# shiyao-li/NextBestPath

Measured on AMD Instinct MI355X. Metric: exploration steps/s (+ NBP maps/s) at 256x256, higher is better.
Workload: dtype f32

## Files before the change

### include/nbp_hip.h

```cpp
#ifndef NBP_HIP_H
#define NBP_HIP_H

#include <stddef.h>
#include <stdint.h>

#ifdef __cplusplus
extern "C" {
#endif

#define NBP_E_ARG      (-1)
#define NBP_E_WS       (-2)
#define NBP_E_SHAPE    (-3)

int nbp_abi_version(void);
int nbp_device_info(char* arch_host, int arch_len, int* cu_count_host);
int nbp_tuning_active(void);
int nbp_tuning_report(char* buf_host, int len);
int nbp_tile_kernel_symbol(int tile, char* buf_host, int len);

#define NBP_N_CONV 48

typedef struct nbp_weights nbp_weights;

size_t nbp_packed_weights_bytes(void);

int nbp_pack_weights(const void* const* w_host_array, const void* const* scale_host_array,
                     const void* const* shift_host_array, void* packed, size_t packed_bytes,
                     void* stream, nbp_weights** handle_out);
void nbp_free_weights(nbp_weights* handle);

size_t nbp_forward_workspace_bytes(int B, int S);

int nbp_forward_f32(const nbp_weights* handle, const float* x, int B, int S, float* out1,
                    float* out2, void* ws, size_t ws_bytes, void* stream);

typedef struct nbp_layer_timing {
    char name[48];
    double flops;
    float ms;
    int tile, split_k;
    long long M;
    int N, K;
} nbp_layer_timing;
int nbp_forward_timed_f32(const nbp_weights* handle, const float* x, int B, int S, float* out1,
                          float* out2, void* ws, size_t ws_bytes, void* stream,
                          nbp_layer_timing* timings_host, int max_entries, int* n_entries_host);

double nbp_forward_flops(int B, int S);

int nbp_pack_weights_bf16(const void* const* w_host_array, const void* const* scale_host_array,
                          const void* const* shift_host_array, void* packed, size_t packed_bytes,
                          void* stream, nbp_weights** handle_out);
// ... 29 lines not shown
int nbp_conv3x3_split_f32(const float* src0, int C0, const float* src1, int C1, int ups, int B, int H, int W,
                          const void* w_planes, const void* wamax, int N, const float* scale, const float* shift, int relu,
                          float* out, const void* amax_in_or_null, void* amax_out_or_null, int split_k, void* ws,
                          size_t ws_bytes, void* stream);
size_t nbp_conv_first_wgrad_workspace_bytes(void);
int nbp_conv_first_wgrad_f32(const float* x_nchw, int B, int H, int W, const float* dy, float* dw, void* ws, size_t ws_bytes, void* stream);
int nbp_prepack_weights_split(const void* descs_dev, int n, void* wamax_words, void* stream);
int nbp_prepack_desc_bytes(void);
int nbp_pack_conv_weight_split_prezeroed(const float* w_oihw, int N, int C, int ksize, int c_total, void* dst_planes,
                                         void* wamax_zeroed, void* stream);
int nbp_pack_conv_weight_split_dgrad_known(const float* w_oihw, int N, int C, int c_total, void* dst_planes, const void* wamax_known,
                                           void* stream);
int nbp_pack_upconv_weight_split_dgrad(const float* w_oihw, int N, int C, void* dst_planes, void* wamax_out, void* stream);
size_t nbp_upconv_split_dgrad_workspace_bytes(int B, int H, int W, int N, int C);
int nbp_upconv3x3_split_dgrad_f32(const float* dy, int N, int B, int H, int W, const void* planes, const void* wamax, int C,
                                  const float* scale, const float* shift, float* dx, const void* amax_in, void* amax_out_or_null,
                                  void* ws, size_t ws_bytes, void* stream);
size_t nbp_upconv_wgrad_split_workspace_bytes(int B, int Hs, int Ws, int C, int N);
int nbp_upconv_wgrad_split_f32(const float* x, int C, int B, int Hs, int Ws, const float* dy, int N, float* dw,
                               const void* amax_x, const void* amax_y, void* ws, size_t ws_bytes, void* stream);
int nbp_conv1x1_split_f32(const float* src, int C, long long M, const void* w_planes, const void* wamax, int N,
                          const float* scale, const float* shift, int relu, float* out, const void* amax_in, void* stream);
int nbp_pack_conv1x1_weight_split_dgrad(const float* w_nc, int N, int C, void* dst_planes, void* wamax_out, void* stream);
int nbp_pack_conv_weight_split_dgrad(const float* w_oihw, int N, int C, int c_total, void* dst_planes, void* wamax_out, void* stream);

int nbp_conv_bn_part_rows(int B, int H, int W);
int nbp_conv3x3_split_bn_f32(const float* src0, int C0, const float* src1, int C1, int ups, int B, int H, int W,
                             const void* w_planes, const void* wamax, int N, const float* scale, const float* shift, int relu,
                             float* out, const void* amax_in_or_null, void* amax_out_or_null, int split_k, void* ws,
                             size_t ws_bytes, double* bn_part, int* bn_rows, void* stream);
int nbp_upconv3x3_split_bn_f32(const float* src, int C, int B, int H, int W, const void* planes_up, const void* wamax_up, int N,
                               const float* scale, const float* shift, int relu, float* out, const void* amax_in_or_null,
                               void* amax_out_or_null, int split_k, void* ws, size_t ws_bytes, double* bn_part, int* bn_rows,
                               void* stream);
int nbp_pack_conv_weight_split_h1(const float* w_oihw, int N, int C, int ksize, const float* scale_or_null, int c_off,
                                  int c_total, void* dst_planes, void* wamax_out, void* stream);
int nbp_pack_conv_weight_split_prezeroed_h1(const float* w_oihw, int N, int C, int ksize, int c_total, void* dst_planes,
                                            void* wamax_zeroed, void* stream);
int nbp_pack_conv_weight_split_dgrad_h1(const float* w_oihw, int N, int C, int c_total, void* dst_planes, void* wamax_out, void* stream);
int nbp_pack_conv_weight_split_dgrad_known_h1(const float* w_oihw, int N, int C, int c_total, void* dst_planes, const void* wamax_known,
                                              void* stream);
int nbp_pack_upconv_weight_split_h1(const float* w_oihw, int N, int C, void* dst_planes, void* wamax_out, void* stream);
int nbp_pack_upconv_weight_split_dgrad_h1(const float* w_oihw, int N, int C, void* dst_planes, void* wamax_out, void* stream);
int nbp_pack_conv1x1_weight_split_dgrad_h1(const float* w_nc, int N, int C, void* dst_planes, void* wamax_out, void* stream);
int nbp_prepack_weights_split_h1(const void* descs_dev, int n, void* wamax_words, void* stream);
int nbp_conv3x3_split_f32_h1(const float* src0, int C0, const float* src1, int C1, int ups, int B, int H, int W,
// ... 390 lines not shown
```

### nextbestpath_amd/_lib.py

```python
from __future__ import annotations

import ctypes as C
import os
import threading

HERE = os.path.dirname(os.path.abspath(__file__))
LIB_PATH = os.path.join(HERE, "libnbp_hip.so")

_vp, _i, _ll, _f, _sz, _d = C.c_void_p, C.c_int, C.c_longlong, C.c_float, C.c_size_t, C.c_double

SIGNATURES = {
    "nbp_abi_version": (_i, []),
    "nbp_device_info": (_i, [C.c_char_p, _i, C.POINTER(_i)]),
    "nbp_tuning_active": (_i, []),
    "nbp_tuning_report": (_i, [C.c_char_p, _i]),
    "nbp_tile_kernel_symbol": (_i, [_i, C.c_char_p, _i]),
    "nbp_packed_weights_bytes": (_sz, []),
    "nbp_pack_weights": (_i, [C.POINTER(_vp), C.POINTER(_vp), C.POINTER(_vp), _vp, _sz, _vp, C.POINTER(_vp)]),
    "nbp_free_weights": (None, [_vp]),
    "nbp_forward_workspace_bytes": (_sz, [_i, _i]),
    "nbp_forward_f32": (_i, [_vp, _vp, _i, _i, _vp, _vp, _vp, _sz, _vp]),
    "nbp_forward_flops": (_d, [_i, _i]),
    "nbp_conv_igemm_f32": (_i, [_vp, _i, _vp, _i, _i, _i, _i, _i, _i, _vp, _i, _vp, _vp, _i, _vp, _i, _i, _vp,
                                _sz, _vp]),
# ... 97 lines not shown
SIGNATURES["nbp_amax_f32"] = (_i, [_vp, _ll, _vp, _vp])
SIGNATURES["nbp_pack_upconv_weight_split"] = (_i, [_vp, _i, _i, _vp, _vp, _vp])
SIGNATURES["nbp_upconv3x3_split_f32"] = (_i, [_vp, _i, _i, _i, _i, _vp, _vp, _i, _vp, _vp, _i, _vp, _vp, _vp, _i, _vp, _sz, _vp])
SIGNATURES["nbp_conv_split_workspace_bytes"] = SIGNATURES["nbp_conv_igemm_workspace_bytes"]
SIGNATURES["nbp_conv_split_planned_workspace_bytes"] = (_sz, [_i, _i, _i, _i, _i, _i, _vp])
SIGNATURES["nbp_conv_split_planned_workspace_bytes_k"] = (_sz, [_i, _i, _i, _i, _i, _i, _i, _vp])
SIGNATURES["nbp_conv3x3_split_f32"] = (_i, [_vp, _i, _vp, _i, _i, _i, _i, _i, _vp, _vp, _i, _vp, _vp, _i, _vp, _vp, _vp, _i, _vp,
                                            _sz, _vp])
SIGNATURES["nbp_pack_upconv_weight_split_dgrad"] = (_i, [_vp, _i, _i, _vp, _vp, _vp])
SIGNATURES["nbp_upconv_split_dgrad_workspace_bytes"] = (_sz, [_i, _i, _i, _i, _i])
SIGNATURES["nbp_upconv3x3_split_dgrad_f32"] = (_i, [_vp, _i, _i, _i, _i, _vp, _vp, _i, _vp, _vp, _vp, _vp, _vp, _vp, _sz, _vp])
SIGNATURES["nbp_upconv_wgrad_split_workspace_bytes"] = (_sz, [_i, _i, _i, _i, _i])
SIGNATURES["nbp_upconv_wgrad_split_f32"] = (_i, [_vp, _i, _i, _i, _i, _vp, _i, _vp, _vp, _vp, _vp, _sz, _vp])
SIGNATURES["nbp_pack_conv_weight_split_prezeroed"] = (_i, [_vp, _i, _i, _i, _i, _vp, _vp, _vp])
SIGNATURES["nbp_pack_conv_weight_split_dgrad_known"] = (_i, [_vp, _i, _i, _i, _vp, _vp, _vp])
SIGNATURES["nbp_prepack_weights_split"] = (_i, [_vp, _i, _vp, _vp])
SIGNATURES["nbp_prepack_desc_bytes"] = (_i, [])
SIGNATURES["nbp_rowscale_amax_f32"] = (_i, [_vp, _vp, _ll, _i, _vp, _vp, _vp])
SIGNATURES["nbp_conv_first_linear_f32"] = (_i, [_vp, _i, _i, _i, _vp, _vp, _vp, _vp, _vp])
SIGNATURES["nbp_conv_first_wgrad_workspace_bytes"] = (_sz, [])
SIGNATURES["nbp_conv_first_wgrad_f32"] = (_i, [_vp, _i, _i, _i, _vp, _vp, _vp, _sz, _vp])
SIGNATURES["nbp_conv1x1_split_f32"] = (_i, [_vp, _i, _ll, _vp, _vp, _i, _vp, _vp, _i, _vp, _vp, _vp])
SIGNATURES["nbp_pack_conv1x1_weight_split_dgrad"] = (_i, [_vp, _i, _i, _vp, _vp, _vp])
SIGNATURES["nbp_pack_conv_weight_split_dgrad"] = (_i, [_vp, _i, _i, _i, _vp, _vp, _vp])
SIGNATURES["nbp_conv_bn_part_rows"] = (_i, [_i, _i, _i])
SIGNATURES["nbp_conv3x3_split_bn_f32"] = (_i, [_vp, _i, _vp, _i, _i, _i, _i, _i, _vp, _vp, _i, _vp, _vp, _i, _vp, _vp, _vp, _i, _vp,
                                               _sz, _vp, C.POINTER(_i), _vp])
SIGNATURES["nbp_upconv3x3_split_bn_f32"] = (_i, [_vp, _i, _i, _i, _i, _vp, _vp, _i, _vp, _vp, _i, _vp, _vp, _vp, _i, _vp, _sz, _vp,
                                                 C.POINTER(_i), _vp])
SIGNATURES["nbp_bn_train_forward_part4_f32"] = (_i, [_vp, _ll, _i, _vp, _vp, _f, _f, _vp, _vp, _i, _vp, _vp, _vp, _vp, _vp, _i, _vp, _i, _vp, _vp])
for _n in ("nbp_pack_conv_weight_split", "nbp_pack_conv_weight_split_prezeroed", "nbp_pack_conv_weight_split_dgrad",
           "nbp_pack_conv_weight_split_dgrad_known", "nbp_pack_upconv_weight_split", "nbp_pack_upconv_weight_split_dgrad",
           "nbp_pack_conv1x1_weight_split_dgrad", "nbp_prepack_weights_split", "nbp_conv3x3_split_f32", "nbp_conv3x3_split_bn_f32",
           "nbp_upconv3x3_split_f32", "nbp_upconv3x3_split_bn_f32", "nbp_upconv3x3_split_dgrad_f32", "nbp_conv1x1_split_f32",
           "nbp_upconv_wgrad_split_f32", "nbp_conv_wgrad_split_f32"):
    SIGNATURES[_n + "_h1"] = SIGNATURES[_n]
SIGNATURES["nbp_conv_igemm_bf16"] = SIGNATURES["nbp_conv_igemm_f32"]
SIGNATURES["nbp_conv_igemm_bf16_workspace_bytes"] = SIGNATURES["nbp_conv_igemm_workspace_bytes"]
SIGNATURES["nbp_pack_conv_weight_bf16"] = SIGNATURES["nbp_pack_conv_weight"]
SIGNATURES["nbp_f32_to_bf16"] = (_i, [_vp, _ll, _vp, _vp])
SIGNATURES["nbp_bf16_to_f32"] = (_i, [_vp, _ll, _vp, _vp])
_fpp, _ipp = C.POINTER(_f), C.POINTER(_i)
SIGNATURES["nbp_scene_fill_workspace_bytes"] = (_sz, [_fpp, _ipp, _i, _ll, _d])
SIGNATURES["nbp_scene_fill_cells_f32"] = (_i, [_vp, _ll, _vp, _fpp, _ipp, _i, _d, _i, C.c_uint, _vp, _vp, _vp, _sz, _vp])
SIGNATURES["nbp_scene_gather_f32"] = (_i, [_vp, _vp, _i, _i, _vp, _ll, _vp, _vp])
SIGNATURES["nbp_scene_coverage_workspace_bytes"] = (_sz, [_fpp, _ipp, _i, _d])
# ... 160 lines not shown
```

### nextbestpath_amd/csrc/nbp_forward.hip

```cpp
#include "common.h"
#include "nbp_internal.h"
#include <stdio.h>
#include <stdlib.h>
#include <string.h>

namespace {

enum Kind { K_FIRST, K_CONV3, K_ATT_G, K_ATT_X, K_PSI, K_FINAL };
struct LayerSpec { Kind kind; int cin, cout, k; };

struct Table {
    LayerSpec L[NBP_N_CONV];
    size_t w_off[NBP_N_CONV];
    size_t s_off[NBP_N_CONV], t_off[NBP_N_CONV];
    size_t total_floats;
    size_t w3_off[NBP_N_CONV];
    size_t w3u_off[NBP_N_CONV];
    bool is_up[NBP_N_CONV];
    int up_rank[NBP_N_CONV];
    size_t total3_bytes;
    size_t wup16_off[NBP_N_CONV], total_up16_bytes;
    size_t w1_off[NBP_N_CONV];
    int gate_rank[NBP_N_CONV];
    Table() {
// ... 74 lines not shown
    for (long long i = (long long)blockIdx.x * blockDim.x + threadIdx.x; i < n; i += (long long)gridDim.x * blockDim.x)
        dst[i] = v;
}
int fill_f32(float* dst, float v, long long n, hipStream_t st) {
    fill_f32_kernel<<<nbp_ew_grid(n, 256), 256, 0, st>>>(dst, v, n);
    return nbp_launch_status();
}

}

struct nbp_weights {
    const void* w[NBP_N_CONV];
    const float* scale[NBP_N_CONV];
    const float* shift[NBP_N_CONV];
    int bf16;
    const void* w3[NBP_N_CONV];
    const unsigned* wamax[NBP_N_CONV];
    const void* wup16[NBP_N_CONV];
    const void* w1[NBP_N_CONV];
    const unsigned* wamax1[NBP_N_CONV];
    const void* w3u[NBP_N_CONV];
    const unsigned* wamax_u[NBP_N_CONV];
    int split;
};

extern "C" int nbp_abi_version(void) {
    NBP_ENTER(); return NBP_ABI_VERSION; }

extern "C" int nbp_device_info(char* arch_host, int arch_len, int* cu_count_host) {
    NBP_ENTER();
    int dev = 0;
    hipError_t e = hipGetDevice(&dev);
    if (e != hipSuccess) return (int)e;
    hipDeviceProp_t p;
    e = hipGetDeviceProperties(&p, dev);
    if (e != hipSuccess) return (int)e;
    if (arch_host && arch_len > 0) { strncpy(arch_host, p.gcnArchName, arch_len - 1); arch_host[arch_len - 1] = 0; }
    if (cu_count_host) *cu_count_host = p.multiProcessorCount;
    return 0;
}

extern "C" size_t nbp_packed_weights_bytes(void) { return table().total_floats * sizeof(float); }

static int pack_weights_impl(const void* const* w_host_array, const void* const* scale_host_array,
                             const void* const* shift_host_array, void* packed, size_t packed_bytes, void* stream,
                             nbp_weights** handle_out, bool bf16, bool split = false) {
    NBP_RETURN_IF(!w_host_array || !scale_host_array || !shift_host_array || !packed || !handle_out, NBP_E_ARG);
    const Table& T = table();
    NBP_RETURN_IF(packed_bytes < T.total_floats * sizeof(float) + (split ? T.total3_bytes : 0) + (bf16 ? T.total_up16_bytes : 0),
                  NBP_E_WS);
    for (int i = 0; i < NBP_N_CONV; ++i) {
        NBP_RETURN_IF(!w_host_array[i] || !scale_host_array[i], NBP_E_ARG);
        NBP_RETURN_IF(T.L[i].kind != K_ATT_X && !shift_host_array[i], NBP_E_ARG);
    }
    hipStream_t st = (hipStream_t)stream;
    float* base = (float*)packed;
    nbp_weights* h = (nbp_weights*)calloc(1, sizeof(nbp_weights));
    NBP_RETURN_IF(!h, NBP_E_ARG);
    h->bf16 = bf16 ? 1 : 0;
    h->split = split ? 1 : 0;
    char* base3 = (char*)packed + T.total_floats * sizeof(float);
    int rc = 0;
    for (int i = 0; i < NBP_N_CONV && !rc; ++i) {
        const LayerSpec& s = T.L[i];
        const float* w = (const float*)w_host_array[i];
        const float* sc = (const float*)scale_host_array[i];
        const float* sh = (const float*)shift_host_array[i];
        float* wd = base + T.w_off[i];
        float* sd = base + T.s_off[i];
        float* td = base + T.t_off[i];
        h->w[i] = wd; h->scale[i] = sd; h->shift[i] = td;
        switch (s.kind) {
            case K_FIRST: case K_FINAL:
                rc = copy_f32(w, wd, (long long)s.cout * s.cin * s.k * s.k, st);
                if (!rc) rc = copy_f32(sc, sd, s.cout, st);
                if (!rc) rc = copy_f32(sh, td, s.cout, st);
                break;
            case K_PSI:
                rc = copy_f32(w, wd, s.cin, st);
                if (!rc) rc = copy_f32(sc, sd, 1, st);
                if (!rc) rc = copy_f32(sh, sd + 1, 1, st);
                if (!rc) rc = copy_f32(sh, td, 1, st);
                break;
// ... 57 lines not shown
                             false);
}

extern "C" int nbp_pack_weights_bf16(const void* const* w_host_array, const void* const* scale_host_array,
                                     const void* const* shift_host_array, void* packed, size_t packed_bytes,
                                     void* stream, nbp_weights** handle_out) {
    NBP_ENTER();
    return pack_weights_impl(w_host_array, scale_host_array, shift_host_array, packed, packed_bytes, stream, handle_out,
                             true);
}

extern "C" size_t nbp_packed_weights_bytes_split(void) { return table().total_floats * sizeof(float) + table().total3_bytes; }
extern "C" int nbp_pack_weights_split(const void* const* w_host_array, const void* const* scale_host_array,
                                      const void* const* shift_host_array, void* packed, size_t packed_bytes,
                                      void* stream, nbp_weights** handle_out) {
    NBP_ENTER();
    return pack_weights_impl(w_host_array, scale_host_array, shift_host_array, packed, packed_bytes, stream, handle_out,
                             false, true);
}

extern "C" size_t nbp_packed_weights_bytes_bf16(void) { return table().total_floats * sizeof(float) + table().total_up16_bytes; }

extern "C" void nbp_free_weights(nbp_weights* handle) { free(handle); }

namespace {

struct Bump {
    char* base; size_t size, off; bool dry;
    template <typename T> T* take(size_t count) {
        size_t bytes = (count * sizeof(T) + 255) / 256 * 256;
        size_t o = off; off += bytes;
        if (dry) return (T*)(uintptr_t)256;
        return (T*)(base + o);
    }
};

struct Timer {
    hipStream_t st;
    nbp_layer_timing* out; int cap; int n;
    hipEvent_t ev[256];
    int nev;
    int begin() {
        nev = 0; n = 0;
        hipError_t e = hipEventCreate(&ev[0]);
        if (e != hipSuccess) return (int)e;
        nev = 1;
// ... 117 lines not shown
                    int H, int ks, int N, void* ws, size_t wsb, hipStream_t st) {
        if (ks == 1 && C1 == C0 && C0 % 64 == 0 && !ups && h->w1[li[0]] && (!o2 || h->w1[li[1]])) {
            const long long M = (long long)B * H * H;
            ConvOperandsSplit s[2];
            for (int g = 0; g < (o2 ? 2 : 1); ++g) {
                const Ops& q = g ? *o2 : o;
                s[g] = ConvOperandsSplit{q.src0, q.src1, h->w1[li[g]], q.scale, q.shift, q.out, nullptr, nullptr, h->wamax1[li[g]], nullptr,
                                         nullptr, nullptr};
                int rc = ctx.ensure(q.src0, M * C0, &s[g].amax0);
                if (!rc) rc = ctx.ensure(q.src1, M * C1, &s[g].amax1);
                if (rc) return rc;
            }
            GatePsi psi;
            for (int g = 0; g < 2; ++g) {
                const int l = li[(g && o2) ? 1 : 0] + 2;
                psi.wpsi[g] = (const float*)h->w[l]; psi.st[g] = h->scale[l]; psi.gated[g] = ctx.gated[(g && o2) ? 1 : 0];
            }
            unsigned* gslot[2] = {nullptr, nullptr};
            if (ctx.gated[0]) for (int g = 0; g < (o2 ? 2 : 1); ++g) psi.gated_amax[g] = gslot[g] = ctx.unbound();
            static const int psi_on_load = nbp_tune_int("NBP_SPLIT_PSI_ON_LOAD", 1);
            const ConvPlan pc = nbp_plan_conv_split(M, C0, (C0 + C0) / 32 * 9, 0, o2 ? 2 : 1, H, H, 3, 0);
            psi.psi_only = psi_on_load && (C0 >= 128 || psi_on_load >= 2) && ctx.gated[0] && gslot[0] && (!o2 || gslot[1]) && pc.tile != 0 &&
                           M * C0 * 4 < (1ll << 31);
            int fused = 0;
            const int rc = nbp_gate1x1_split_launch_g(s[0], o2 ? &s[1] : nullptr, C0, M, N, 1, st, ctx.gated[0] ? &psi : nullptr, &fused);
            if (fused) {
                ctx.gated_taken = true;
                for (int g = 0; g < (o2 ? 2 : 1); ++g) {
                    if (gslot[g]) ctx.bind(ctx.gated[g], gslot[g]);
                    else ctx.alias(ctx.gated[g], (g ? *o2 : o).src1);
                    if (psi.psi_only) { ctx.psi_key[g] = ctx.gated[g]; ctx.psi_x[g] = (g ? *o2 : o).src1; }
                }
            }
            return rc;
        }
        const ConvPlan p = nbp_plan_conv_split((long long)B * H * H, N, (C0 + C1) / 32 * ks * ks, 0, o2 ? 2 : 1, H, H, ks, ups);
        if (!p.tile) return PathF32::conv(ctx, h, li, o, o2, C0, C1, ups, B, H, ks, N, ws, wsb, st);
        const long long hw = (long long)B * (ups ? H / 2 : H) * (ups ? H / 2 : H);
        ConvOperandsSplit s[2];
        for (int g = 0; g < (o2 ? 2 : 1); ++g) {
            const Ops& q = g ? *o2 : o;
            s[g] = ConvOperandsSplit{q.src0, q.src1, h->w3[li[g]], q.scale, q.shift, q.out, nullptr, nullptr, h->wamax[li[g]], nullptr,
                                     h->w3u[li[g]], h->wamax_u[li[g]]};
            int rc = ctx.ensure(q.src0, hw * C0, &s[g].amax0);
            if (!rc && C1) rc = ctx.ensure(q.src1, hw * C1, &s[g].amax1);
            if (rc) return rc;
// ... 339 lines not shown
```

### nextbestpath_amd/csrc/nbp_internal.h

```cpp
#pragma once
#include "common.h"

typedef unsigned short bf16_t;

enum { NBP_TILE_AUTO = 0, NBP_TILE_128x128 = 1, NBP_TILE_256x64 = 2, NBP_TILE_256x32 = 3, NBP_TILE_128x64 = 4,
       NBP_TILE_64x128 = 5,
       NBP_TILE_HALO_128 = 6, NBP_TILE_HALO_64 = 7,
       NBP_TILE_HALO4_128 = 8, NBP_TILE_HALO4_64 = 9,
       NBP_TILE_SPLIT_HALO_64 = 10, NBP_TILE_SPLIT_UP = 11,
       NBP_TILE_HALO_UP_128 = 12, NBP_TILE_HALO_UP_64 = 13,
       NBP_TILE_RESERVED_14 = 14,
       NBP_TILE_SPLIT_HALO_R8 = 15, NBP_TILE_SPLIT_UP_R8 = 16,
       NBP_TILE_SPLIT_UP_DGRAD = 17,
       NBP_TILE_SPLIT_HALO_128 = 18,
       NBP_TILE_SPLIT_GATE = 19 };
struct TileInfo { int bm, bn; };
struct ConvPlan { int tile; int split_k; int chunks_per_split; };

struct IgemmArgs {
    const float* src0;
    const float* src1;
    int C0, C1;
    int cc0;
    int ups;
// ... 30 lines not shown

struct ConvOperandsSplit {
    const float* src0; const float* src1; const void* planes; const float* scale; const float* shift; float* out;
    const unsigned* amax0; const unsigned* amax1; const unsigned* wamax; unsigned* amax_out;
    const void* planes_up; const unsigned* wamax_up;
    const float* psi0 = nullptr;
};
ConvPlan nbp_plan_conv_split(long long M, int N, int chunks_total, int split_k, int groups, int H, int W, int ksize, int ups = 0);
int nbp_pack_upconv_weight_split_launch(const float* w_oihw, int N, int C, void* dst, unsigned* wamax_out, hipStream_t st, int one = 0);
struct ConvHead { const float* w; const float* scale; const float* shift; float* out; };
int nbp_conv_split_launch_g(const ConvOperandsSplit& o, const ConvOperandsSplit* o2, int C0, int C1, int ups, int B, int H, int W,
                            int ksize, int N, int relu, int split_k, void* ws, size_t ws_bytes, hipStream_t st,
                            float* const* pool_out = nullptr, int* pooled = nullptr, const struct ConvHead* head = nullptr,
                            int* headed = nullptr, double* bn_part = nullptr, int* bn_rows = nullptr, int one = 0);
int nbp_pack_conv_weight_split_launch(const float* w_oihw, int N, int C, int ksize, const float* scale_or_null, int c_off,
                                      int c_total, void* dst, unsigned* wamax_out, hipStream_t st, int one = 0);
int nbp_amax_launch(const float* x, long long n, unsigned* amax_inout, hipStream_t st);
int nbp_wgrad_split_launch(const float* src0, int C0, const float* src1, int C1, int ups, int B, int H, int W, const float* dy, int N,
                           int n_tiles, int splits, unsigned* amax3, const unsigned* amax0_in, const unsigned* amax1_in,
                           const unsigned* amaxy_in, float* part, hipStream_t st);
int nbp_pack_gate_weight_split_launch(const float* wg, const float* scale_g, const float* wx, const float* scale_x, int N, int C,
                                      void* dst, unsigned* wamax_out, hipStream_t st);
struct GatePsi { const float* wpsi[2]; const float* st[2]; float* gated[2]; unsigned* gated_amax[2] = {nullptr, nullptr};
                 int psi_only = 0; };
int nbp_gate1x1_split_launch_g(const ConvOperandsSplit& o, const ConvOperandsSplit* o2, int C, long long M, int N, int relu,
                               hipStream_t st, const GatePsi* psi = nullptr, int* fused = nullptr);
int nbp_conv_first_amax_launch(const float* x_nchw, int B, int H, int W, const float* w_oihw, const float* scale, const float* shift,
                               float* out_nhwc, unsigned* amax_out, int* did_amax, hipStream_t st);

struct ConvOperandsH { const bf16_t* src0; const bf16_t* src1; const bf16_t* wpk; const float* scale; const float* shift; bf16_t* out;
                       const bf16_t* wpk_up; };
ConvPlan nbp_plan_conv_bf16(long long M, int N, int chunks_total, int tile, int split_k, int groups, int H = 0, int W = 0,
                            int ksize = 0, int ups = 0);
int nbp_pack_upconv_weight_bf16_launch(const float* w_oihw, int N, int C, bf16_t* dst, hipStream_t st);
struct GatePsiH { const float* wpsi[2]; const float* st[2]; bf16_t* gated[2]; };
int nbp_conv_igemm_bf16_launch_g(const ConvOperandsH& o, const ConvOperandsH* o2, int C0, int C1, int ups, int B, int H,
                                 int W, int ksize, int N, int relu, int split_k, int tile, void* ws, size_t ws_bytes,
                                 hipStream_t st, bf16_t* const* pool_out = nullptr, int* pooled = nullptr,
                                 const struct ConvHead* head = nullptr, int* headed = nullptr, const GatePsiH* psi = nullptr,
                                 int* psi_fused = nullptr);
int nbp_conv_first_bf16_launch(const float* x_nchw, int B, int H, int W, const float* w_oihw, const float* scale,
                               const float* shift, bf16_t* out_nhwc, hipStream_t st);
int nbp_maxpool2_bf16_launch(const bf16_t* in, int B, int H, int W, int C, bf16_t* out, hipStream_t st);
int nbp_psi_gate_bf16_launch(const bf16_t* q, int F, const float* w_psi, const float* s_t2, const bf16_t* x, int C,
                             long long M, bf16_t* out, hipStream_t st);
int nbp_final_1x1_bf16_launch(const bf16_t* in, int B, int H, int W, int C, const float* w_oc, int n_out,
                              const float* scale, const float* shift, int sigmoid, float* out_nchw, hipStream_t st);
// ... 1 lines not shown
```

### nextbestpath_amd/csrc/nbp_split.hip

```cpp
#include "common.h"
#include "nbp_internal.h"
#include <cstdlib>

namespace {

typedef _Float16 f16x8 __attribute__((ext_vector_type(8)));
typedef _Float16 f16x2 __attribute__((ext_vector_type(2)));
typedef unsigned u32x4 __attribute__((ext_vector_type(4)));
typedef unsigned u32x2 __attribute__((ext_vector_type(2)));
typedef __attribute__((address_space(3))) void* lds_ptr_t;

constexpr int SPLIT_EXP = 14;
__host__ __device__ inline int amax_exponent(unsigned bits) {
    if (!bits) return SPLIT_EXP;
    int e = (int)((bits >> 23) & 255u) - 127;
    return e < -100 ? -100 : (e > 100 ? 100 : e);
}
__host__ __device__ inline float pow2f(int e) {
    union { unsigned u; float f; } v;
    v.u = (unsigned)(127 + e) << 23;
    return v.f;
}

__device__ __forceinline__ void split_pair(float x0, float x1, unsigned& h, unsigned& l) {
// ... 499 lines not shown

#ifdef NBP_DBG_TS
extern "C" int nbp_dbg_read(unsigned long long* host, unsigned* n) {
    hipDeviceSynchronize();
    hipMemcpyFromSymbol(n, HIP_SYMBOL(nbp_dbg_n), sizeof(unsigned));
    return (int)hipMemcpyFromSymbol(host, HIP_SYMBOL(nbp_dbg_ts), sizeof(unsigned long long) * 8192);
}
#endif

struct GateArgs {
    SplitOps g[2];
    int C, N, relu;
    int C1;
    long long M;
    unsigned bytes0, bytesw;
    int groups;
    const float* wpsi[2];
    const float* st[2];
    float* gated[2];
    unsigned* gated_amax[2];
    int psi_only;
};

template <bool ONE, int TN, bool PSI>
__global__ __launch_bounds__(256, 2) void gate1x1_h2_kernel(GateArgs a) {
    const SplitOps& o = a.g[blockIdx.z];
    constexpr int BN = TN * 32;
    constexpr int WST = (ONE ? 4 : 8) * BN * 16;
    constexpr int WI = WST / 1024;
    extern __shared__ __attribute__((aligned(16))) char wbuf[];
    const int tid = threadIdx.x, lane = tid & 63, wave = tid >> 6;
    const long long m = (long long)blockIdx.x * 128 + wave * 32 + (lane & 31);
    const int n0 = blockIdx.y * BN, khalf = lane >> 5;
    const unsigned ma0 = read_amax(o.amax0), ma1 = o.amax1 ? read_amax(o.amax1) : 0u;
    const int ea = amax_exponent(ma0 > ma1 ? ma0 : ma1), ew = amax_exponent(*o.wamax);
    const float sa = pow2f(SPLIT_EXP - ea);
    const int einv = ea + ew - 2 * SPLIT_EXP;
    const __amdgpu_buffer_rsrc_t rs0 = __builtin_amdgcn_make_buffer_rsrc(const_cast<float*>(o.src0), 0, a.bytes0, 0x00020000);
    const __amdgpu_buffer_rsrc_t rs1 = __builtin_amdgcn_make_buffer_rsrc(const_cast<float*>(o.src1 ? o.src1 : o.src0), 0, a.bytes0, 0x00020000);
    const __amdgpu_buffer_rsrc_t rsw = __builtin_amdgcn_make_buffer_rsrc(const_cast<void*>(o.planes), 0, a.bytesw, 0x00020000);
    constexpr unsigned OOB = 0x80000000u;
    const int stages0 = a.C >> 5, stages = stages0 + (a.C1 >> 5);
    const unsigned prow = m < a.M ? (unsigned)(m * a.C) * 4u : OOB;

    constexpr int D = 4;
    u32x4 xr[D][2][2];
    auto load_x = [&](int st, int slot) {
        const bool first = st < stages0;
        const unsigned cb = (unsigned)((first ? st : st - stages0) * 32 + khalf * 8) * 4u;
#pragma unroll
        for (int ks = 0; ks < 2; ++ks)
#pragma unroll
            for (int h = 0; h < 2; ++h) {
                const unsigned off = (prow == OOB || st >= stages) ? OOB : prow + cb + ks * 64 + h * 16;
                xr[slot][ks][h] = first ? __builtin_amdgcn_raw_buffer_load_b128(rs0, off, 0, 0) : __builtin_amdgcn_raw_buffer_load_b128(rs1, off, 0, 0);
            }
    };
    auto issue_w = [&](int st) {
        char* dst = wbuf + (st & 1) * WST;
#pragma unroll
        for (int k = 0; k < (WI + 3) / 4; ++k) {
            const int q = wave + 4 * k;
            if (q < WI) {
                constexpr int PER = BN / 64 > 0 ? BN / 64 : 1;
                const int r8 = BN >= 64 ? q / PER : q * 2 + (lane >> 5), nb = BN >= 64 ? q - (q / PER) * PER : 0;
                const int row = BN >= 64 ? nb * 64 + lane : (lane & 31);
                const int ks = ONE ? r8 >> 1 : r8 >> 2, r4 = ONE ? r8 & 1 : r8 & 3;
                const unsigned woff = (unsigned)((((long long)(2 * st + ks) * (ONE ? 2 : 4) + r4) * a.N + n0 + row) * 16);
                __builtin_amdgcn_raw_ptr_buffer_load_lds(rsw, (lds_ptr_t)(dst + q * 1024), 16, woff, 0, 0, 0);
            }
        }
    };

    f32x16 acc[TN];
#pragma unroll
    for (int j = 0; j < TN; ++j)
#pragma unroll
        for (int r = 0; r < 16; ++r) acc[j][r] = 0.f;

    issue_w(0);
#pragma unroll
    for (int d = 0; d < D - 1; ++d) load_x(d, d);
    asm volatile("s_waitcnt vmcnt(0)" ::: "memory");
    __syncthreads();
    for (int base = 0; base < stages; base += D) {
#pragma unroll
        for (int u = 0; u < D; ++u) {
            const int st = base + u;
            if (st + 1 < stages) issue_w(st + 1);
            load_x(st + D - 1, (u + D - 1) % D);
            const char* Bt = wbuf + (st & 1) * WST + khalf * (BN * 16) + (lane & 31) * 16;
            if (st < stages)
#pragma unroll
            for (int ks = 0; ks < 2; ++ks) {
                const f32x4 v0 = __builtin_bit_cast(f32x4, xr[u][ks][0]), v1 = __builtin_bit_cast(f32x4, xr[u][ks][1]);
                if constexpr (ONE) {
                    const u32x4 xh = u32x4{hi_pair(v0[0] * sa, v0[1] * sa), hi_pair(v0[2] * sa, v0[3] * sa), hi_pair(v1[0] * sa, v1[1] * sa),
                                           hi_pair(v1[2] * sa, v1[3] * sa)};
#pragma unroll
                    for (int j = 0; j < TN; ++j) {
                        const u32x4 wh = *reinterpret_cast<const u32x4*>(Bt + (ks * 2) * (BN * 16) + j * 512);
                        acc[j] = __builtin_amdgcn_mfma_f32_32x32x16_f16(__builtin_bit_cast(f16x8, xh), __builtin_bit_cast(f16x8, wh), acc[j], 0, 0, 0);
                    }
                    continue;
                }
                unsigned h0, l0, h1, l1, h2, l2, h3, l3;
                split_pair(v0[0] * sa, v0[1] * sa, h0, l0); split_pair(v0[2] * sa, v0[3] * sa, h1, l1);
                split_pair(v1[0] * sa, v1[1] * sa, h2, l2); split_pair(v1[2] * sa, v1[3] * sa, h3, l3);
                const u32x4 xh = u32x4{h0, h1, h2, h3}, xl = u32x4{l0, l1, l2, l3};
#pragma unroll
                for (int j = 0; j < TN; ++j) {
                    const u32x4 wh = *reinterpret_cast<const u32x4*>(Bt + ((ks * 2 + 0) * 2) * (BN * 16) + j * 512);
                    const u32x4 wl = *reinterpret_cast<const u32x4*>(Bt + ((ks * 2 + 1) * 2) * (BN * 16) + j * 512);
                    acc[j] = __builtin_amdgcn_mfma_f32_32x32x16_f16(__builtin_bit_cast(f16x8, xl), __builtin_bit_cast(f16x8, wh), acc[j], 0, 0, 0);
                    acc[j] = __builtin_amdgcn_mfma_f32_32x32x16_f16(__builtin_bit_cast(f16x8, xh), __builtin_bit_cast(f16x8, wl), acc[j], 0, 0, 0);
                    acc[j] = __builtin_amdgcn_mfma_f32_32x32x16_f16(__builtin_bit_cast(f16x8, xh), __builtin_bit_cast(f16x8, wh), acc[j], 0, 0, 0);
                }
            }
            asm volatile("s_waitcnt vmcnt(4)" ::: "memory");
            __syncthreads();
        }
    }
    const long long mw = (long long)blockIdx.x * 128 + wave * 32;
    if constexpr (PSI) {
        float p[16];
#pragma unroll
        for (int r = 0; r < 16; ++r) p[r] = 0.f;
#pragma unroll
        for (int j = 0; j < TN; ++j) {
            const int n = j * 32 + (lane & 31);
            const float sc = o.scale[n], sh = o.shift[n], wp = a.wpsi[blockIdx.z][n];
#pragma unroll
            for (int r = 0; r < 16; ++r) {
                float v = ldexpf(acc[j][r], einv) * sc + sh;
                if (a.relu) v = fmaxf(v, 0.f);
                p[r] = fmaf(v, wp, p[r]);
            }
        }
        float p8[8], p4[4], p2[2];
        {
            const bool up = lane & 16;
#pragma unroll
            for (int i = 0; i < 8; ++i) p8[i] = (up ? p[8 + i] : p[i]) + __shfl_xor(up ? p[i] : p[8 + i], 16);
        }
        {
            const bool up = lane & 8;
#pragma unroll
            for (int i = 0; i < 4; ++i) p4[i] = (up ? p8[4 + i] : p8[i]) + __shfl_xor(up ? p8[i] : p8[4 + i], 8);
        }
        {
            const bool up = lane & 4;
#pragma unroll
            for (int i = 0; i < 2; ++i) p2[i] = (up ? p4[2 + i] : p4[i]) + __shfl_xor(up ? p4[i] : p4[2 + i], 4);
        }
        float dot;
        {
            const bool up = lane & 2;
            dot = (up ? p2[1] : p2[0]) + __shfl_xor(up ? p2[0] : p2[1], 2);
        }
        dot += __shfl_xor(dot, 1);
        const float z = dot * a.st[blockIdx.z][0] + a.st[blockIdx.z][1];
        const float psi = 1.f / (1.f + expf(-z));
        float* psil = reinterpret_cast<float*>(wbuf) + wave * 32;
        const int r = (lane & 31) >> 1;
        if (!(lane & 1)) {
            const int pix = (r & 3) + 8 * (r >> 2) + 4 * khalf;
            psil[pix] = psi;
            if (a.psi_only && mw + pix < a.M) a.gated[blockIdx.z][mw + pix] = psi;
        }
        asm volatile("s_waitcnt lgkmcnt(0)" ::: "memory");
        const int C4 = a.C >> 2, total = 32 * C4;
        const f32x4* x4 = reinterpret_cast<const f32x4*>(o.src1) + mw * C4;
        f32x4* g4 = reinterpret_cast<f32x4*>(a.gated[blockIdx.z]) + mw * C4;
        const long long lim = (a.M - mw) * C4;
        float gmx = 0.f;
#pragma unroll 1
        for (int i0 = lane; i0 < total; i0 += 256) {
            f32x4 v[4];
#pragma unroll
            for (int u = 0; u < 4; ++u) { const int i = i0 + 64 * u; if (i < total && i < lim) v[u] = x4[i]; }
#pragma unroll
            for (int u = 0; u < 4; ++u) {
                const int i = i0 + 64 * u;
                if (i < total && i < lim) {
                    const float ps = psil[i / C4];
                    const f32x4 g = v[u] * ps;
                    if (!a.psi_only) g4[i] = g;
                    gmx = fmaxf(fmaxf(gmx, fmaxf(fabsf(g[0]), fabsf(g[1]))), fmaxf(fabsf(g[2]), fabsf(g[3])));
                }
            }
        }
        if (a.gated_amax[blockIdx.z]) wave_amax(gmx, a.gated_amax[blockIdx.z]);
    } else {
#pragma unroll
    for (int j = 0; j < TN; ++j) {
        const int n = n0 + j * 32 + (lane & 31);
        const float sc = o.scale[n], sh = o.shift[n];
#pragma unroll
        for (int r = 0; r < 16; ++r) {
            const long long mm = mw + (r & 3) + 8 * (r >> 2) + 4 * khalf;
            if (mm < a.M) {
                float v = ldexpf(acc[j][r], einv) * sc + sh;
                if (a.relu) v = fmaxf(v, 0.f);
                o.out[mm * a.N + n] = v;
            }
        }
    }
    }
}

struct WgradSplitArgs {
// ... 994 lines not shown
        pack_upconv_h2_kernel<true><<<grid, 256, 0, st>>>(w_oihw, N, C, wamax_out, (unsigned short*)dst);
    } else {
        pack_upconv_h2_kernel<<<min(grid, 256), 256, 0, st>>>(w_oihw, N, C, wamax_out, nullptr);
        pack_upconv_h2_kernel<<<grid, 256, 0, st>>>(w_oihw, N, C, wamax_out, (unsigned short*)dst);
    }
    return nbp_launch_status();
}

int nbp_pack_gate_weight_split_launch(const float* wg, const float* scale_g, const float* wx, const float* scale_x, int N, int C,
                                      void* dst, unsigned* wamax_out, hipStream_t st) {
    NBP_RETURN_IF(!wg || !wx || !dst || !wamax_out, NBP_E_ARG);
    NBP_RETURN_IF(N < 32 || N % 32 || C < 32 || C % 32, NBP_E_SHAPE);
    hipError_t e = hipMemsetAsync(wamax_out, 0, sizeof(unsigned), st);
    if (e != hipSuccess) return (int)e;
    const long long total = (long long)N * C;
    const int grid = min(nbp_ew_grid(total, 256), 256);
    amax_kernel<<<grid, 256, 0, st>>>(wg, total, scale_g, C, wamax_out, 1u);
    amax_kernel<<<grid, 256, 0, st>>>(wx, total, scale_x, C, wamax_out, 1u);
    pack_conv_weight_h2_kernel<<<nbp_ew_grid(total, 256), 256, 0, st>>>(wg, N, C, 1, scale_g, 0, wamax_out, (unsigned short*)dst);
    pack_conv_weight_h2_kernel<<<nbp_ew_grid(total, 256), 256, 0, st>>>(wx, N, C, 1, scale_x, C, wamax_out, (unsigned short*)dst);
    return nbp_launch_status();
}

int nbp_gate1x1_split_launch_g(const ConvOperandsSplit& o, const ConvOperandsSplit* o2, int C, long long M, int N, int relu,
                               hipStream_t st, const GatePsi* psi, int* fused) {
    const int groups = o2 ? 2 : 1;
    NBP_RETURN_IF(!o.src0 || !o.src1 || !o.planes || !o.scale || !o.shift || !o.out || !o.amax0 || !o.amax1 || !o.wamax, NBP_E_ARG);
    NBP_RETURN_IF(o2 && (!o2->src0 || !o2->src1 || !o2->planes || !o2->out || !o2->amax0 || !o2->amax1 || !o2->wamax), NBP_E_ARG);
    NBP_RETURN_IF(C < 64 || C % 64 || N < 32 || N % 32 || M < 1, NBP_E_SHAPE);
    const long long b0 = M * C * 4, bw = 2ll * C * N * 4;
    NBP_RETURN_IF(b0 >= (1ll << 31) || bw >= (1ll << 31), NBP_E_SHAPE);
    GateArgs a;
    for (int g = 0; g < 2; ++g) {
        const ConvOperandsSplit& s = (g && o2) ? *o2 : o;
        a.g[g] = SplitOps{s.src0, s.src1, s.planes, s.scale, s.shift, s.out, s.amax0, s.amax1, s.wamax, nullptr, nullptr, nullptr, {nullptr, nullptr}, nullptr};
        const int gi = g < groups ? g : 0;
        a.wpsi[g] = psi ? psi->wpsi[gi] : nullptr; a.st[g] = psi ? psi->st[gi] : nullptr; a.gated[g] = psi ? psi->gated[gi] : nullptr;
        a.gated_amax[g] = psi ? psi->gated_amax[gi] : nullptr;
    }
    a.psi_only = psi ? psi->psi_only : 0;
    a.C = C; a.C1 = C; a.N = N; a.relu = relu; a.M = M; a.bytes0 = (unsigned)b0; a.bytesw = (unsigned)bw; a.groups = groups;
    int bn = N % 128 == 0 ? 128 : (N % 64 == 0 ? 64 : 32);
    static const int allow_psi = nbp_tune_int("NBP_GATE_PSI", 1);
    const bool psi_wants_128 = allow_psi && psi && N == 128 && psi->wpsi[0] && psi->st[0] && psi->gated[0];
    if (bn == 128 && nbp_cdiv(M, 128) * (N / 128) * groups < 512 && !psi_wants_128) bn = 64;
    const bool with_psi = allow_psi && psi && bn == N && psi->wpsi[0] && psi->st[0] && psi->gated[0] &&
                          (groups == 1 || (psi->wpsi[1] && psi->st[1] && psi->gated[1]));
    if (fused) *fused = with_psi;
    dim3 grid((unsigned)nbp_cdiv(M, 128), (unsigned)(N / bn), (unsigned)groups);
    const size_t smem = 2 * (size_t)8 * bn * 16;
    {
        char nm[64];
        snprintf(nm, sizeof(nm), "gate1x1_h2_kernel<false, %d, %s>", bn / 32, with_psi ? "true" : "false");
        nbp_note_kernel_symbol(NBP_TILE_SPLIT_GATE, nm);
    }
    if (with_psi) {
        if (bn == 128) gate1x1_h2_kernel<false, 4, true><<<grid, 256, smem, st>>>(a);
        else if (bn == 64) gate1x1_h2_kernel<false, 2, true><<<grid, 256, smem, st>>>(a);
        else gate1x1_h2_kernel<false, 1, true><<<grid, 256, smem, st>>>(a);
    } else if (bn == 128) gate1x1_h2_kernel<false, 4, false><<<grid, 256, smem, st>>>(a);
    else if (bn == 64) gate1x1_h2_kernel<false, 2, false><<<grid, 256, smem, st>>>(a);
    else gate1x1_h2_kernel<false, 1, false><<<grid, 256, smem, st>>>(a);
    return nbp_launch_status();
}

int nbp_upconv_dgrad_split_launch(const float* dy, int N, int B, int H, int W, const void* planes, const unsigned* wamax,
                                  const unsigned* amax_in, int C, const float* scale, const float* shift, float* out, unsigned* amax_out,
                                  int split_k, void* ws, size_t ws_bytes, hipStream_t st, int one = 0) {
    NBP_RETURN_IF(!dy || !planes || !wamax || !amax_in || !scale || !shift || !out, NBP_E_ARG);
    NBP_RETURN_IF(B < 1 || N < 16 || N % 16 || C < 64 || C % 64, NBP_E_SHAPE);
    const int tw = split_tile_width(H, W, C, 3);
    NBP_RETURN_IF(!tw, NBP_E_SHAPE);
    SplitArgs a;
    for (int g = 0; g < 2; ++g)
        a.g[g] = SplitOps{dy, nullptr, planes, scale, shift, out, amax_in, nullptr, wamax, amax_out, nullptr, nullptr, {nullptr, nullptr}, nullptr, nullptr};
    a.C0 = N; a.C1 = 0; a.ups = 0; a.H = H; a.W = W; a.Hs = 2 * H; a.Ws = 2 * W; a.N = C; a.relu = 0; a.groups = 1;
    a.M = (long long)B * H * W;
    const long long b0 = (long long)B * 4 * H * W * N * 4, bw = 64ll * N * C;
    NBP_RETURN_IF(b0 >= (1ll << 31) || bw >= (1ll << 31), NBP_E_SHAPE);
// ... 172 lines not shown
                                                                                             (unsigned short*)dst_planes, 1);
    return nbp_launch_status();
}
extern "C" int nbp_pack_conv_weight_split_prezeroed(const float* w_oihw, int N, int C, int ksize, int c_total, void* dst_planes,
                                                    void* wamax_zeroed, void* stream) {
    NBP_ENTER();
    return pack_conv_weight_split_prezeroed_impl<false>(w_oihw, N, C, ksize, c_total, dst_planes, wamax_zeroed, stream);
}
extern "C" int nbp_pack_conv_weight_split_dgrad_known(const float* w_oihw, int N, int C, int c_total, void* dst_planes,
                                                      const void* wamax_known, void* stream) {
    NBP_ENTER();
    return pack_conv_weight_split_dgrad_known_impl<false>(w_oihw, N, C, c_total, dst_planes, wamax_known, stream);
}
extern "C" int nbp_pack_conv_weight_split_prezeroed_h1(const float* w_oihw, int N, int C, int ksize, int c_total, void* dst_planes,
                                                       void* wamax_zeroed, void* stream) {
    NBP_ENTER();
    return pack_conv_weight_split_prezeroed_impl<true>(w_oihw, N, C, ksize, c_total, dst_planes, wamax_zeroed, stream);
}
extern "C" int nbp_pack_conv_weight_split_dgrad_known_h1(const float* w_oihw, int N, int C, int c_total, void* dst_planes,
                                                         const void* wamax_known, void* stream) {
    NBP_ENTER();
    return pack_conv_weight_split_dgrad_known_impl<true>(w_oihw, N, C, c_total, dst_planes, wamax_known, stream);
}
extern "C" int nbp_amax_f32(const float* x, long long n, void* amax_inout, void* stream) {
    NBP_ENTER();
    NBP_RETURN_IF(!x || !amax_inout || n < 0, NBP_E_ARG);
    return nbp_amax_launch(x, n, (unsigned*)amax_inout, (hipStream_t)stream);
}

extern "C" size_t nbp_conv_split_workspace_bytes(int B, int H, int W, int N, int split_k) {
    const int sk = split_k == 1 ? 0 : (split_k <= 0 ? 16 : split_k);
    return 256 + (size_t)sk * B * H * W * N * sizeof(float);
}

extern "C" size_t nbp_conv_split_planned_workspace_bytes_k(int B, int H, int W, int C, int N, int ups, int split_k, int* split_k_out);
extern "C" size_t nbp_conv_split_planned_workspace_bytes(int B, int H, int W, int C, int N, int ups, int* split_k_out) {
    return nbp_conv_split_planned_workspace_bytes_k(B, H, W, C, N, ups, 0, split_k_out);
}
extern "C" size_t nbp_conv_split_planned_workspace_bytes_k(int B, int H, int W, int C, int N, int ups, int split_k, int* split_k_out) {
    if (B < 1 || H < 1 || W < 1 || C < 32 || N < 1) return 0;
    const ConvPlan p = nbp_plan_conv_split((long long)B * H * W, N, C / 32 * 9, split_k, 1, H, W, 3, ups ? 1 : 0);
    if (split_k_out) *split_k_out = p.tile ? p.split_k : 0;
    const int sk = (p.tile && p.split_k > 1) ? p.split_k : 0;
    return 256 + (size_t)sk * B * H * W * N * sizeof(float);
}

// ... 289 lines not shown
```

Before: 2356.

## Fuse gated-output amax and store into attention-gate GEMM tail

Adds TAIL variants of the gate 1x1 kernel with PSI. They compute the abs-max of the skip input during the k-loop and scale it by psi, so the post-GEMM loop that re-reads src1 only to build the amax can be skipped. For small channel counts (RING variants), the whole x operand is kept in the register ring and the gated output is written straight from registers, with no second global read. The default picks tail 1 when psi_only is set and otherwise uses the old path, and adds test APIs plus an env knob. The risks are register pressure and the extra vmcnt(0) waits at the ring tail.

```diff
diff --git a/include/nbp_hip.h b/include/nbp_hip.h
--- a/include/nbp_hip.h
+++ b/include/nbp_hip.h
@@ -28,6 +28,7 @@
                      const void* const* shift_host_array, void* packed, size_t packed_bytes,
                      void* stream, nbp_weights** handle_out);
 void nbp_free_weights(nbp_weights* handle);
+int nbp_weights_set_gate_tail(nbp_weights* handle, int tail);
 
 size_t nbp_forward_workspace_bytes(int B, int S);
 
@@ -103,6 +104,12 @@
 int nbp_conv1x1_split_f32(const float* src, int C, long long M, const void* w_planes, const void* wamax, int N,
                           const float* scale, const float* shift, int relu, float* out, const void* amax_in, void* stream);
 int nbp_pack_conv1x1_weight_split_dgrad(const float* w_nc, int N, int C, void* dst_planes, void* wamax_out, void* stream);
+int nbp_pack_gate_weight_split(const float* wg, const float* scale_g, const float* wx, const float* scale_x, int N, int C,
+                               void* dst_planes, void* wamax_out, void* stream);
+int nbp_gate_psi_split_f32(int groups, const float* const* g, const float* const* x, int C, long long M, const void* const* planes,
+                           const void* const* wamax, int N, const float* const* scale, const float* const* shift,
+                           const void* const* amax_g, const void* const* amax_x, const float* const* wpsi, const float* const* st2,
+                           float* const* q_scratch, float* const* gated, void* const* gated_amax, int psi_only, int tail, void* stream);
 int nbp_pack_conv_weight_split_dgrad(const float* w_oihw, int N, int C, int c_total, void* dst_planes, void* wamax_out, void* stream);
 
 int nbp_conv_bn_part_rows(int B, int H, int W);
diff --git a/nextbestpath_amd/_lib.py b/nextbestpath_amd/_lib.py
--- a/nextbestpath_amd/_lib.py
+++ b/nextbestpath_amd/_lib.py
@@ -143,6 +143,9 @@
 SIGNATURES["nbp_conv_first_wgrad_f32"] = (_i, [_vp, _i, _i, _i, _vp, _vp, _vp, _sz, _vp])
 SIGNATURES["nbp_conv1x1_split_f32"] = (_i, [_vp, _i, _ll, _vp, _vp, _i, _vp, _vp, _i, _vp, _vp, _vp])
 SIGNATURES["nbp_pack_conv1x1_weight_split_dgrad"] = (_i, [_vp, _i, _i, _vp, _vp, _vp])
+SIGNATURES["nbp_weights_set_gate_tail"] = (_i, [_vp, _i])
+SIGNATURES["nbp_pack_gate_weight_split"] = (_i, [_vp, _vp, _vp, _vp, _i, _i, _vp, _vp, _vp])
+SIGNATURES["nbp_gate_psi_split_f32"] = (_i, [_i, _vp, _vp, _i, _ll, _vp, _vp, _i, _vp, _vp, _vp, _vp, _vp, _vp, _vp, _vp, _vp, _i, _i, _vp])
 SIGNATURES["nbp_pack_conv_weight_split_dgrad"] = (_i, [_vp, _i, _i, _i, _vp, _vp, _vp])
 SIGNATURES["nbp_conv_bn_part_rows"] = (_i, [_i, _i, _i])
 SIGNATURES["nbp_conv3x3_split_bn_f32"] = (_i, [_vp, _i, _vp, _i, _i, _i, _i, _i, _vp, _vp, _i, _vp, _vp, _i, _vp, _vp, _vp, _i, _vp,
diff --git a/nextbestpath_amd/csrc/nbp_forward.hip b/nextbestpath_amd/csrc/nbp_forward.hip
--- a/nextbestpath_amd/csrc/nbp_forward.hip
+++ b/nextbestpath_amd/csrc/nbp_forward.hip
@@ -120,6 +120,7 @@
     const void* w3u[NBP_N_CONV];
     const unsigned* wamax_u[NBP_N_CONV];
     int split;
+    int gate_tail;
 };
 
 extern "C" int nbp_abi_version(void) {
@@ -157,6 +158,7 @@
     NBP_RETURN_IF(!h, NBP_E_ARG);
     h->bf16 = bf16 ? 1 : 0;
     h->split = split ? 1 : 0;
+    h->gate_tail = -1;
     char* base3 = (char*)packed + T.total_floats * sizeof(float);
     int rc = 0;
     for (int i = 0; i < NBP_N_CONV && !rc; ++i) {
@@ -260,6 +262,12 @@
 extern "C" size_t nbp_packed_weights_bytes_bf16(void) { return table().total_floats * sizeof(float) + table().total_up16_bytes; }
 
 extern "C" void nbp_free_weights(nbp_weights* handle) { free(handle); }
+extern "C" int nbp_weights_set_gate_tail(nbp_weights* handle, int tail) {
+    NBP_ENTER();
+    NBP_RETURN_IF(!handle || tail < -1 || tail > 2, NBP_E_ARG);
+    handle->gate_tail = tail;
+    return 0;
+}
 
 namespace {
 
@@ -423,6 +431,7 @@
             const ConvPlan pc = nbp_plan_conv_split(M, C0, (C0 + C0) / 32 * 9, 0, o2 ? 2 : 1, H, H, 3, 0);
             psi.psi_only = psi_on_load && (C0 >= 128 || psi_on_load >= 2) && ctx.gated[0] && gslot[0] && (!o2 || gslot[1]) && pc.tile != 0 &&
                            M * C0 * 4 < (1ll << 31);
+            psi.tail = h->gate_tail;
             int fused = 0;
             const int rc = nbp_gate1x1_split_launch_g(s[0], o2 ? &s[1] : nullptr, C0, M, N, 1, st, ctx.gated[0] ? &psi : nullptr, &fused);
             if (fused) {
diff --git a/nextbestpath_amd/csrc/nbp_internal.h b/nextbestpath_amd/csrc/nbp_internal.h
--- a/nextbestpath_amd/csrc/nbp_internal.h
+++ b/nextbestpath_amd/csrc/nbp_internal.h
@@ -76,7 +76,8 @@
 int nbp_pack_gate_weight_split_launch(const float* wg, const float* scale_g, const float* wx, const float* scale_x, int N, int C,
                                       void* dst, unsigned* wamax_out, hipStream_t st);
 struct GatePsi { const float* wpsi[2]; const float* st[2]; float* gated[2]; unsigned* gated_amax[2] = {nullptr, nullptr};
-                 int psi_only = 0; };
+                 int psi_only = 0;
+                 int tail = -1; };
 int nbp_gate1x1_split_launch_g(const ConvOperandsSplit& o, const ConvOperandsSplit* o2, int C, long long M, int N, int relu,
                                hipStream_t st, const GatePsi* psi = nullptr, int* fused = nullptr);
 int nbp_conv_first_amax_launch(const float* x_nchw, int B, int H, int W, const float* w_oihw, const float* scale, const float* shift,
diff --git a/nextbestpath_amd/csrc/nbp_split.hip b/nextbestpath_amd/csrc/nbp_split.hip
--- a/nextbestpath_amd/csrc/nbp_split.hip
+++ b/nextbestpath_amd/csrc/nbp_split.hip
@@ -545,8 +545,10 @@
     int psi_only;
 };
 
-template <bool ONE, int TN, bool PSI>
+template <bool ONE, int TN, bool PSI, int TAIL = 0>
 __global__ __launch_bounds__(256, 2) void gate1x1_h2_kernel(GateArgs a) {
+    static_assert(TAIL == 0 || (PSI && (TAIL == 1 || TAIL == 2 || TAIL == 4)), "register tails belong to the PSI form");
+    constexpr bool RING = TAIL >= 2;
     const SplitOps& o = a.g[blockIdx.z];
     constexpr int BN = TN * 32;
     constexpr int WST = (ONE ? 4 : 8) * BN * 16;
@@ -555,7 +557,10 @@
     const int tid = threadIdx.x, lane = tid & 63, wave = tid >> 6;
     const long long m = (long long)blockIdx.x * 128 + wave * 32 + (lane & 31);
     const int n0 = blockIdx.y * BN, khalf = lane >> 5;
-    const unsigned ma0 = read_amax(o.amax0), ma1 = o.amax1 ? read_amax(o.amax1) : 0u;
+    unsigned ma0 = read_amax(o.amax0), ma1 = o.amax1 ? read_amax(o.amax1) : 0u;
+    if constexpr (TAIL != 0) {
+        ma0 = __builtin_amdgcn_readfirstlane(ma0); ma1 = __builtin_amdgcn_readfirstlane(ma1);
+    }
     const int ea = amax_exponent(ma0 > ma1 ? ma0 : ma1), ew = amax_exponent(*o.wamax);
     const float sa = pow2f(SPLIT_EXP - ea);
     const int einv = ea + ew - 2 * SPLIT_EXP;
@@ -563,7 +568,7 @@
     const __amdgpu_buffer_rsrc_t rs1 = __builtin_amdgcn_make_buffer_rsrc(const_cast<float*>(o.src1 ? o.src1 : o.src0), 0, a.bytes0, 0x00020000);
     const __amdgpu_buffer_rsrc_t rsw = __builtin_amdgcn_make_buffer_rsrc(const_cast<void*>(o.planes), 0, a.bytesw, 0x00020000);
     constexpr unsigned OOB = 0x80000000u;
-    const int stages0 = a.C >> 5, stages = stages0 + (a.C1 >> 5);
+    const int stages0 = RING ? TAIL : a.C >> 5, stages = RING ? 2 * TAIL : stages0 + (a.C1 >> 5);
     const unsigned prow = m < a.M ? (unsigned)(m * a.C) * 4u : OOB;
 
     constexpr int D = 4;
@@ -601,6 +606,7 @@
 #pragma unroll
         for (int r = 0; r < 16; ++r) acc[j][r] = 0.f;
 
+    float xmax = 0.f;
     issue_w(0);
 #pragma unroll
     for (int d = 0; d < D - 1; ++d) load_x(d, d);
@@ -611,12 +617,17 @@
         for (int u = 0; u < D; ++u) {
             const int st = base + u;
             if (st + 1 < stages) issue_w(st + 1);
-            load_x(st + D - 1, (u + D - 1) % D);
+            const bool ahead = !RING || st + D - 1 < stages;
+            if (ahead) load_x(st + D - 1, (u + D - 1) % D);
             const char* Bt = wbuf + (st & 1) * WST + khalf * (BN * 16) + (lane & 31) * 16;
             if (st < stages)
 #pragma unroll
             for (int ks = 0; ks < 2; ++ks) {
                 const f32x4 v0 = __builtin_bit_cast(f32x4, xr[u][ks][0]), v1 = __builtin_bit_cast(f32x4, xr[u][ks][1]);
+                if constexpr (TAIL != 0)
+                    if (st >= stages0)
+#pragma unroll
+                        for (int e = 0; e < 4; ++e) xmax = fmaxf(fmaxf(xmax, fabsf(v0[e])), fabsf(v1[e]));
                 if constexpr (ONE) {
                     const u32x4 xh = u32x4{hi_pair(v0[0] * sa, v0[1] * sa), hi_pair(v0[2] * sa, v0[3] * sa), hi_pair(v1[0] * sa, v1[1] * sa),
                                            hi_pair(v1[2] * sa, v1[3] * sa)};
@@ -640,12 +651,15 @@
                     acc[j] = __builtin_amdgcn_mfma_f32_32x32x16_f16(__builtin_bit_cast(f16x8, xh), __builtin_bit_cast(f16x8, wh), acc[j], 0, 0, 0);
                 }
             }
-            asm volatile("s_waitcnt vmcnt(4)" ::: "memory");
+            if (ahead) asm volatile("s_waitcnt vmcnt(4)" ::: "memory");
+            else asm volatile("s_waitcnt vmcnt(0)" ::: "memory");
             __syncthreads();
         }
     }
     const long long mw = (long long)blockIdx.x * 128 + wave * 32;
     if constexpr (PSI) {
+        float* xml = reinterpret_cast<float*>(wbuf) + 128 + wave * 64;
+        if constexpr (TAIL != 0) xml[lane] = xmax;
         float p[16];
 #pragma unroll
         for (int r = 0; r < 16; ++r) p[r] = 0.f;
@@ -692,11 +706,29 @@
             if (a.psi_only && mw + pix < a.M) a.gated[blockIdx.z][mw + pix] = psi;
         }
         asm volatile("s_waitcnt lgkmcnt(0)" ::: "memory");
-        const int C4 = a.C >> 2, total = 32 * C4;
+        float gmx = 0.f;
+        if constexpr (TAIL != 0) {
+            const float ps = psil[lane & 31];
+            gmx = fmaxf(gmx, fabsf(fmaxf(xml[lane], xml[lane ^ 32]) * ps));
+            if constexpr (RING) {
+                const __amdgpu_buffer_rsrc_t rsg = __builtin_amdgcn_make_buffer_rsrc(a.gated[blockIdx.z], 0, a.bytes0, 0x00020000);
+#pragma unroll
+                for (int s1 = 0; s1 < TAIL; ++s1)
+#pragma unroll
+                    for (int ks = 0; ks < 2; ++ks)
+#pragma unroll
+                        for (int h = 0; h < 2; ++h) {
+                            const unsigned off = prow + (unsigned)(s1 * 32 + khalf * 8) * 4u + ks * 64 + h * 16;
+                            const f32x4 g = __builtin_bit_cast(f32x4, xr[(TAIL + s1) % D][ks][h]) * ps;
+                            if (prow != OOB) __builtin_amdgcn_raw_buffer_store_b128(__builtin_bit_cast(u32x4, g), rsg, off, 0, 0);
+                        }
+            }
+        }
+        const bool reread = !RING && !(TAIL != 0 && a.psi_only);
+        const int C4 = a.C >> 2, total = reread ? 32 * C4 : 0;
         const f32x4* x4 = reinterpret_cast<const f32x4*>(o.src1) + mw * C4;
         f32x4* g4 = reinterpret_cast<f32x4*>(a.gated[blockIdx.z]) + mw * C4;
         const long long lim = (a.M - mw) * C4;
-        float gmx = 0.f;
 #pragma unroll 1
         for (int i0 = lane; i0 < total; i0 += 256) {
             f32x4 v[4];
@@ -709,7 +741,7 @@
                     const float ps = psil[i / C4];
                     const f32x4 g = v[u] * ps;
                     if (!a.psi_only) g4[i] = g;
-                    gmx = fmaxf(fmaxf(gmx, fmaxf(fabsf(g[0]), fabsf(g[1]))), fmaxf(fabsf(g[2]), fabsf(g[3])));
+                    if constexpr (TAIL == 0) gmx = fmaxf(fmaxf(gmx, fmaxf(fabsf(g[0]), fabsf(g[1]))), fmaxf(fabsf(g[2]), fabsf(g[3])));
                 }
             }
         }
@@ -1750,6 +1782,8 @@
     return nbp_launch_status();
 }
 
+constexpr int GATE_TAIL_PSI_ONLY = 1, GATE_TAIL_WRITTEN = 0;
+
 int nbp_gate1x1_split_launch_g(const ConvOperandsSplit& o, const ConvOperandsSplit* o2, int C, long long M, int N, int relu,
                                hipStream_t st, const GatePsi* psi, int* fused) {
     const int groups = o2 ? 2 : 1;
@@ -1777,12 +1811,22 @@
     if (fused) *fused = with_psi;
     dim3 grid((unsigned)nbp_cdiv(M, 128), (unsigned)(N / bn), (unsigned)groups);
     const size_t smem = 2 * (size_t)8 * bn * 16;
+    static const int tail_knob = nbp_tune_int("NBP_GATE_TAIL", -1);
+    int tail = psi && psi->tail >= 0 ? psi->tail : tail_knob;
+    if (tail < 0) tail = a.psi_only ? GATE_TAIL_PSI_ONLY : GATE_TAIL_WRITTEN;
+    int kt = !with_psi ? 0 : tail <= 0 ? 0 : (tail == 1 || a.psi_only) ? 1 : (bn == 32 && C == 64) ? 2 : (bn == 64 && C == 128) ? 4 : 1;
     {
         char nm[64];
-        snprintf(nm, sizeof(nm), "gate1x1_h2_kernel<false, %d, %s>", bn / 32, with_psi ? "true" : "false");
+        snprintf(nm, sizeof(nm), "gate1x1_h2_kernel<false, %d, %s, %d>", bn / 32, with_psi ? "true" : "false", kt);
         nbp_note_kernel_symbol(NBP_TILE_SPLIT_GATE, nm);
     }
-    if (with_psi) {
+    if (with_psi && kt == 1) {
+        if (bn == 128) gate1x1_h2_kernel<false, 4, true, 1><<<grid, 256, smem, st>>>(a);
+        else if (bn == 64) gate1x1_h2_kernel<false, 2, true, 1><<<grid, 256, smem, st>>>(a);
+        else gate1x1_h2_kernel<false, 1, true, 1><<<grid, 256, smem, st>>>(a);
+    } else if (with_psi && kt == 2) gate1x1_h2_kernel<false, 1, true, 2><<<grid, 256, smem, st>>>(a);
+    else if (with_psi && kt == 4) gate1x1_h2_kernel<false, 2, true, 4><<<grid, 256, smem, st>>>(a);
+    else if (with_psi) {
         if (bn == 128) gate1x1_h2_kernel<false, 4, true><<<grid, 256, smem, st>>>(a);
         else if (bn == 64) gate1x1_h2_kernel<false, 2, true><<<grid, 256, smem, st>>>(a);
         else gate1x1_h2_kernel<false, 1, true><<<grid, 256, smem, st>>>(a);
@@ -2001,6 +2045,36 @@
     NBP_ENTER();
     return pack_conv_weight_split_dgrad_known_impl<true>(w_oihw, N, C, c_total, dst_planes, wamax_known, stream);
 }
+extern "C" int nbp_pack_gate_weight_split(const float* wg, const float* scale_g, const float* wx, const float* scale_x, int N, int C,
+                                          void* dst_planes, void* wamax_out, void* stream) {
+    NBP_ENTER();
+    return nbp_pack_gate_weight_split_launch(wg, scale_g, wx, scale_x, N, C, dst_planes, (unsigned*)wamax_out, (hipStream_t)stream);
+}
+extern "C" int nbp_gate_psi_split_f32(int groups, const float* const* g, const float* const* x, int C, long long M,
+                                      const void* const* planes, const void* const* wamax, int N, const float* const* scale,
+                                      const float* const* shift, const void* const* amax_g, const void* const* amax_x,
+                                      const float* const* wpsi, const float* const* st2, float* const* q_scratch, float* const* gated,
+                                      void* const* gated_amax, int psi_only, int tail, void* stream) {
+    NBP_ENTER();
+    NBP_RETURN_IF(groups < 1 || groups > 2 || !g || !x || !planes || !wamax || !scale || !shift || !amax_g || !amax_x || !wpsi || !st2 ||
+                  !q_scratch || !gated || !gated_amax, NBP_E_ARG);
+    NBP_RETURN_IF(N != 32 && N != 64 && N != 128, NBP_E_SHAPE);
+    NBP_RETURN_IF(psi_only && M * C * 4 >= (1ll << 31), NBP_E_SHAPE);
+    ConvOperandsSplit s[2];
+    GatePsi psi;
+    for (int k = 0; k < 2; ++k) {
+        const int i = k < groups ? k : 0;
+        NBP_RETURN_IF(!wpsi[i] || !st2[i] || !gated[i] || !gated_amax[i], NBP_E_ARG);
+        s[k] = ConvOperandsSplit{g[i], x[i], planes[i], scale[i], shift[i], q_scratch[i], (const unsigned*)amax_g[i], (const unsigned*)amax_x[i],
+                                 (const unsigned*)wamax[i], nullptr, nullptr, nullptr};
+        psi.wpsi[k] = wpsi[i]; psi.st[k] = st2[i]; psi.gated[k] = gated[i]; psi.gated_amax[k] = (unsigned*)gated_amax[i];
+    }
+    psi.psi_only = psi_only ? 1 : 0;
+    psi.tail = tail;
+    int fused = 0;
+    const int rc = nbp_gate1x1_split_launch_g(s[0], groups == 2 ? &s[1] : nullptr, C, M, N, 1, (hipStream_t)stream, &psi, &fused);
+    return rc ? rc : (fused ? 0 : NBP_E_SHAPE);
+}
 extern "C" int nbp_amax_f32(const float* x, long long n, void* amax_inout, void* stream) {
     NBP_ENTER();
     NBP_RETURN_IF(!x || !amax_inout || n < 0, NBP_E_ARG);
```

Measured after the change: 2365, median of 6. No clear change (+0.4%).
